# Pixie8888/R3DFSSeg

Hardware: AMD Instinct MI355X
Metric: episodes/sec S3DIS 2-way 5-shot 2048-pt (MPTI+attention, train step: forward+backward+grad all-reduce+Adam) (higher is better)
Workload: dtype f32 (index-free GEMMs -- self-attention, 1x1 convolutions, weight gradients, the EdgeConv backward's edge GEMMs -- as bf16x3 split products on the bf16 MFMA with fp32 accumulate; every index-deciding result: fp32)

## Files before the change

include/r3d.h:

```cpp
#ifndef R3D_H
#define R3D_H
#include <stdint.h>

#ifdef __cplusplus
extern "C" {
#endif

const char* r3d_last_error_string(void);
int r3d_abi_version(void);
int r3d_debug_poison_lds(unsigned pattern, unsigned* sink , void* stream);
int r3d_debug_set_cg_spmv_lds_min_blocks(int min_blocks);
int r3d_set_matrix_arith(int mode);
int r3d_get_matrix_arith(void);
int r3d_debug_set_gemm_bx3(int mask);

int r3d_cm_to_pm(const float* in , int B, int C, int N, float* out , long ld, void* stream);
int r3d_pm_to_cm(const float* in , long ld, int B, int C, int N, float* out , void* stream);
int r3d_pm_to_cm_pitched(const float* in, long ld, int B, int C, int N, float* out , long pitch, void* stream);
long r3d_cm_pitch(int N);
int r3d_copy_cols(const float* src, long ld_src, float* dst, long ld_dst, long M, int C, void* stream);

int r3d_sqnorm(const float* x, long ldx, long rows, int C, float* out, void* stream);
long r3d_knn_norm_ws_words(int B, int N);
int r3d_knn_topk(const float* x, long ldx, const float* x_cm, int B, int N, int C, int k, int mode,
// ... 38 lines not shown
                                int32_t* ws, long ws_words, long ws_stride, int flags, void* stream);

long r3d_lp_ws_words(int n_cap, int kp1);
int r3d_lp_ws_offsets(int n_cap, int kp1, long* out6);
int r3d_label_propagate(const float* nodes, long ldn, int D, const int32_t* nbr, int kp1, const float* Y,
                        const int32_t* n_dev, const int32_t* n_proto_dev, int n_cap, float sigma, float alpha,
                        int max_iter, float tol, float* Z, int32_t* ws, long ws_words, int32_t* stats_out, void* stream);

int r3d_label_propagate_batched(int n_ep, const float* nodes, long ldn, int D, const int32_t* nbr, int kp1, const float* Y,
                                const int32_t* n_dev, const int32_t* n_proto_dev, long desc_stride, int n_cap, float sigma,
                                float alpha, int max_iter, float tol, float* Z, int32_t* ws, long ws_words, long ws_stride,
                                int32_t* stats_out, long stats_stride, void* stream);
long r3d_graph_weights_verify_words(int n_cap, int kp1);
int r3d_graph_weights_verify(int n_ep, const float* nodes, long ldn, int D, const int32_t* n_dev, long desc_stride, int n_cap,
                             int kp1, float sigma, int32_t* ws, long ws_words, long ws_stride, float* scratch,
                             int32_t* mismatch_out, void* stream);

int r3d_label_propagate_solve_batched(int n_ep, const float* Y, const int32_t* n_dev, long desc_stride, int n_cap, int kp1,
                                      float alpha, int max_iter, float tol, float* Z, int32_t* ws, long ws_words,
                                      long ws_stride, int32_t* stats_out, long stats_stride, void* stream);

int r3d_graph_set_lp_budget(void* graph, void* graph_exec, int budget, int* n_cg);

int r3d_query_logits_ce(const float* Z, const int32_t* n_proto_dev, int n_q, int N, int n_classes,
                        const int64_t* labels , float* logits ,
                        float* loss_out , int32_t* pred_out , void* stream);

int r3d_query_logits_ce_batched(int n_ep, const float* Z, long z_ep_rows, const int32_t* n_proto_dev, long desc_stride, int n_q,
                                int N, int n_classes, const int64_t* labels, float* logits, float* loss_out, int32_t* pred_out,
                                void* stream);

int r3d_pointwise_conv_acc(const float* X, long ldx, const float* W, long M, int K, int Co, const float* scale,
                           const float* shift, int act, float* Out, long ldo, void* stream);
long r3d_pointwise_conv_stats_ws_words(long M, int Co);
int r3d_pointwise_conv_stats(const float* X, long ldx, const float* W, long M, int K, int Co, float* Out, long ldo,
                             float* sums_out , float* ws, void* stream);
int r3d_pointwise_conv_stats2(const float* X, long ldx, const float* W, long M, int K, int Co, float* Out, long ldo,
                              long M_first, float* sums_a , float* sums_b , float* ws, void* stream);
int r3d_pointwise_conv_stats_seg(const float* X, long ldx, const float* W, long M, int K, int Co, float* Out, long ldo,
                                 long rows_a, long rows_b, float* sums_out, float* ws, void* stream);
int r3d_colreduce(const float* part , int chunks, int C, float* sums_out , void* stream);
int r3d_colreduce_seg(const float* part, int count_a, int count_b, int n_seg, int C, float* sums_out , void* stream);
long r3d_colstats_ws_words(long M, int C);
int r3d_colstats(const float* X, long ldx, const float* DY, long lddy, long M, int C, int mode, const float* scale,
                 const float* shift, const float* mean, const float* invstd, int act, float* sums_out ,
                 float* ws, void* stream);
int r3d_bn_fold(const float* sums, double count, int C, const float* gamma, const float* beta, float eps,
                float momentum, float* running_mean , float* running_var , float* mean, float* invstd,
                float* scale, float* shift, float* rec , const int32_t* rec_index_dev , long rec_stride,
                void* stream);
long r3d_colstats_seg_ws_words(long M, int C, long rows_a, long rows_b);
int r3d_colstats_seg(const float* X, long ldx, const float* DY, long lddy, long M, int C, long rows_a, long rows_b, int mode,
                     const float* scale, const float* shift, const float* mean, const float* invstd, long bn_stride, int act,
                     float* sums_out , float* ws, void* stream);
int r3d_bn_fold_seg(const float* sums , int n_seg, double count_a, double count_b, int C, const float* gamma,
                    const float* beta, float eps, float momentum, float* running_mean , float* running_var ,
                    float* mean, float* invstd, float* scale, float* shift, long bn_stride, float* rec ,
                    const int32_t* rec_index_dev , long rec_stride, void* stream);
int r3d_affine_act_seg(const float* Z, long ldz, long M, int C, long rows_a, long rows_b, const float* scale, const float* shift,
                       long bn_stride, int act, float* Y, long ldy, void* stream);
int r3d_bn_bwd_apply_seg(const float* Z, long ldz, const float* DY, long lddy, long M, int C, long rows_a, long rows_b,
                         const float* scale, const float* shift, const float* mean, const float* invstd, long bn_stride, int act,
                         const float* sums , double count_a, double count_b, float* DZ, long lddz, void* stream);
int r3d_bn_running_update(const float* rec, int n_records, long rec_stride, int C, float momentum,
                          const float* bias , float* running_mean,
                          float* running_var, void* stream);
int r3d_affine_act(const float* Z, long ldz, long M, int C, const float* scale, const float* shift, int act, float* Y,
                   long ldy, void* stream);
int r3d_bn_bwd_apply(const float* Z, long ldz, const float* DY, long lddy, long M, int C, const float* scale,
                     const float* shift, const float* mean, const float* invstd, int act, const float* sums,
                     double count, float* DZ, long lddz, void* stream);
long r3d_gemm_tn_ws_words(long M, int Ca, int Cb);
int r3d_gemm_tn(const float* A, long lda, const float* B, long ldb, long M, int Ca, int Cb, float alpha, float* out,
                int accumulate, float* ws, void* stream);
int r3d_add_cols(const float* src, long ld_src, float* dst, long ld_dst, long M, int C, void* stream);

long r3d_edgeconv_train_ws_words(int B, int N);
int r3d_edge_stats1(const float* PQ, const int32_t* idx, int B, int N, int K, int clouds_a, int clouds_b,
                    float* sums_out , float* esum , float* ws,
                    void* stream);
int r3d_edgeconv_train_fwd_minmax(const float* PQ, const int32_t* idx, const float* s1, const float* t1, long bn_stride,
                                  const float* W2, int B, int N, int K, int clouds_a, int clouds_b, float* zmax, float* zmin,
                                  int32_t* argmax, int32_t* argmin, float* sums_out , float* ws, void* stream);
int r3d_edge_select(float* zmax , const float* zmin, int32_t* argmax ,
                    const int32_t* argmin, const float* s2, const float* t2, long bn_stride, long M, long rows_a, long rows_b,
                    float* out, long ldo, void* stream);
long r3d_edge_reverse_ws_words(int B, int N, int K);
int r3d_edge_reverse(const int32_t* idx, int B, int N, int K, int32_t* rev_ws, long ws_words, void* stream);
int r3d_edgeconv_bwd(const float* PQ, const int32_t* idx, const float* s1, const float* t1, const float* mean1,
                     const float* invstd1, const float* W2, const float* s2, const float* t2, const float* mean2,
                     const float* invstd2, long bn_stride, const float* bn2_sums, const float* dout, long lddo,
                     const int32_t* argmax, const float* zwin , const float* esum , int B, int N, int K,
                     int clouds_a, int clouds_b, float* DY1 , float* BE ,
                     const int32_t* rev_ws , float* dW2, float* bn1_sums, float* dPQ,
                     float* ws, void* stream);

int r3d_attention_fwd_train(const float* qkv, long ld, int B, int N, float* out, long ldo, float* lse_out, float p_drop,
                            unsigned seed, const unsigned* seed_dev, float* ws , void* stream);
int r3d_attention_bwd(const float* qkv, long ld, int B, int N, const float* O, long ldo, const float* dO, long lddo,
                      const float* lse, float p_drop, unsigned seed, const unsigned* seed_dev, float q_scale, float* dqkv,
                      long ldd, float* ws , void* stream);
int r3d_attention_bwd_ws(const float* qkv, long ld, int B, int N, const float* O, long ldo, const float* dO, long lddo,
                         const float* lse, float p_drop, unsigned seed, const unsigned* seed_dev, float q_scale,
                         float* dqkv, long ldd, float* ws, int ws_holds_packed_qkv, void* stream);

long r3d_attention_ws_words_ep(int B, int N, int seed_group);
int r3d_attention_fwd_train_ep(const float* qkv, long ld, int B, int N, float* out, long ldo, float* lse_out, float p_drop,
                               unsigned seed, const unsigned* seed_dev, int seed_group, float* ws, void* stream);
int r3d_attention_bwd_ep(const float* qkv, long ld, int B, int N, const float* O, long ldo, const float* dO, long lddo,
                         const float* lse, float p_drop, unsigned seed, const unsigned* seed_dev, int seed_group, float q_scale,
                         float* dqkv, long ldd, float* ws, int ws_holds_packed_qkv, void* stream);

long r3d_attention_ws_words_ep_d(int B, int N, int seed_group, int D);
int r3d_attention_fwd_train_ep_d(const float* qkv, long ld, int B, int N, float* out, long ldo, float* lse_out, float p_drop,
                                 unsigned seed, const unsigned* seed_dev, int seed_group, int D, float* ws, void* stream);
int r3d_attention_bwd_ep_d(const float* qkv, long ld, int B, int N, const float* O, long ldo, const float* dO, long lddo,
                           const float* lse, float p_drop, unsigned seed, const unsigned* seed_dev, int seed_group, int D,
                           float q_scale, float* dqkv, long ldd, float* ws, int ws_holds_packed_qkv, void* stream);

int r3d_ce_grad(const float* Z, const int32_t* n_proto_dev, int n_cap, int n_query_pts, int n_classes,
                const int64_t* labels, const float* gscale_dev, float* G, void* stream);
int r3d_label_propagate_bwd(const float* nodes, long ldn, int D, int kp1, const float* Z, const float* G,
                            const int32_t* n_dev, int n_cap, float sigma, float alpha, int max_iter, float tol, float* lam,
                            float* dnodes, long ldd, int32_t* ws, long ws_words, int32_t* stats_out, void* stream);
int r3d_head_prototypes_bwd(const float* dnodes, long ldd, int n_way, int k_shot, int N, int D, int n_query_pts,
                            const int32_t* desc, const int32_t* assign, const int32_t* cluster_count, const int32_t* ws,
                            float* dsfeat, long lds_, float* dqfeat, long ldq, void* stream);

int r3d_ce_grad_batched(int n_ep, const float* Z, const int32_t* n_proto_dev, long desc_stride, int n_cap, int n_query_pts,
                        int n_classes, const int64_t* labels, const float* gscale_dev, float* G, void* stream);
int r3d_label_propagate_bwd_batched(int n_ep, const float* nodes, long ldn, int D, int kp1, const float* Z, const float* G,
                                    const int32_t* n_dev, long desc_stride, int n_cap, float sigma, float alpha, int max_iter,
                                    float tol, float* lam, float* dnodes, long ldd, int32_t* ws, long ws_words, long ws_stride,
                                    int32_t* stats_out, long stats_stride, void* stream);
int r3d_head_prototypes_bwd_batched(int n_ep, const float* dnodes, long ldd, long nodes_ep_rows, int n_way, int k_shot, int N,
                                    int D, int n_query_pts, const int32_t* desc, long desc_stride, const int32_t* assign,
                                    long assign_stride, const int32_t* cluster_count, long ccount_stride, const int32_t* ws,
                                    long ws_stride, float* dsfeat, long lds_, long dsfeat_ep_rows, float* dqfeat, long ldq,
                                    long dqfeat_ep_rows, void* stream);

long r3d_contrast_ws_words(int n_way, int k_shot, int N);
int r3d_contrast_fwd(const float* feat, long ldf, int D, const int32_t* support_y, const int32_t* support_flag, int n_way,
                     int k_shot, int N, const float* W, const float* bias, float temp, float* loss_out, float* ws,
                     long ws_words, void* stream);
int r3d_contrast_bwd(int D, int n_way, int k_shot, int N, const float* gscale_dev, float* dfeat, long ldd, float* dW,
                     float* db, float* ws, void* stream);
int r3d_contrast_fwd_batched(int n_ep, const float* feat, long ldf, long feat_ep_rows, int D, const int32_t* support_y,
                             const int32_t* support_flag, int n_way, int k_shot, int N, const float* W, const float* bias,
                             float temp, float* loss_out, float* ws, long ws_words, long ws_stride, void* stream);
int r3d_contrast_bwd_batched(int n_ep, int D, int n_way, int k_shot, int N, const float* gscale_dev, float* dfeat, long ldd,
                             long dfeat_ep_rows, float* dW, float* db, float* ws, long ws_stride, void* stream);
int r3d_train_metrics_batched(int n_ep, const int32_t* pred, const int64_t* query_y, const int64_t* gt_query_y, int n_query_pts,
                              const float* Z, long z_ep_rows, const int32_t* desc, long desc_stride, const int32_t* proto_ws,
                              long pws_stride, const int32_t* assign, long assign_stride, const int32_t* gt_support_y, int n_way,
                              int k_shot, int N, float* out4 , void* stream);
int r3d_train_metrics(const int32_t* pred, const int64_t* query_y, const int64_t* gt_query_y, int n_query_pts, const float* Z,
                      const int32_t* desc, const int32_t* proto_ws, const int32_t* assign, const int32_t* gt_support_y,
                      int n_way, int k_shot, int N, float* out4, void* stream);

long r3d_clean_ws_words(int n_way, int k_shot);
int r3d_clean_shot_detect(const float* feat , long ldf, int D, const float* support_x ,
                          int Cin, const int32_t* support_y, int n_way, int k_shot, int N, int32_t* shot_keep,
                          float* dbg_cos_sum , int32_t* ws, void* stream);

int r3d_clean_shot_detect_batched(int n_ep, const float* feat, long ldf, long feat_ep_rows, int D, const float* support_x,
                                  int Cin, const int32_t* support_y, int n_way, int k_shot, int N, int32_t* shot_keep,
// ... 14 lines not shown
```

r3dfsseg_amd/_lib.py:

```python
import ctypes
import os
import re

_HERE = os.path.dirname(os.path.abspath(__file__))
LIB_PATH = os.environ.get("R3D_LIB") or os.path.join(_HERE, "libr3d_hip.so")
HEADER_PATH = os.path.join(os.path.dirname(_HERE), "include", "r3d.h")

c_f = ctypes.c_void_p
c_i = ctypes.c_int
c_l = ctypes.c_long
c_fl = ctypes.c_float
c_d = ctypes.c_double
c_u = ctypes.c_uint

_SIGS = {
    "r3d_last_error_string": (ctypes.c_char_p, []),
    "r3d_abi_version": (c_i, []),
    "r3d_cm_to_pm": (c_i, [c_f, c_i, c_i, c_i, c_f, c_l, c_f]),
    "r3d_pm_to_cm": (c_i, [c_f, c_l, c_i, c_i, c_i, c_f, c_f]),
    "r3d_pm_to_cm_pitched": (c_i, [c_f, c_l, c_i, c_i, c_i, c_f, c_l, c_f]),
    "r3d_cm_pitch": (c_l, [c_i]),
    "r3d_copy_cols": (c_i, [c_f, c_l, c_f, c_l, c_l, c_i, c_f]),
    "r3d_sqnorm": (c_i, [c_f, c_l, c_l, c_i, c_f, c_f]),
    "r3d_knn_topk": (c_i, [c_f, c_l, c_f, c_i, c_i, c_i, c_i, c_i, c_f, c_f, c_f, c_f, c_f, c_f, c_f]),
    "r3d_pointwise_conv": (c_i, [c_f, c_l, c_f, c_l, c_i, c_i, c_f, c_f, c_i, c_f, c_l, c_f]),
    "r3d_edgeconv_fwd": (c_i, [c_f, c_f, c_f, c_f, c_f, c_f, c_l, c_i, c_i, c_i, c_f, c_f]),
    "r3d_attention_ws_words": (c_l, [c_i, c_i]),
    "r3d_knn_norm_ws_words": (c_l, [c_i, c_i]),
    "r3d_attention_fwd": (c_i, [c_f, c_l, c_i, c_i, c_f, c_l, c_f, c_f, c_f]),
    "r3d_head_desc_words": (c_i, []),
    "r3d_debug_poison_lds": (c_i, [c_u, c_f, c_f]),
    "r3d_debug_set_cg_spmv_lds_min_blocks": (c_i, [c_i]),
    "r3d_debug_set_gemm_bx3": (c_i, [c_i]),
    "r3d_set_matrix_arith": (c_i, [c_i]),
    "r3d_get_matrix_arith": (c_i, []),
    "r3d_head_max_k": (c_i, []),
    "r3d_fps_sample_count_table": (c_i, [c_i, c_i, c_f, c_f]),
    "r3d_head_proto_ws_words": (c_l, [c_i, c_i, c_i]),
    "r3d_head_proto_ws_offsets": (c_i, [c_i, c_i, c_i, ctypes.POINTER(c_l)]),
    "r3d_head_prototypes": (c_i, [c_f, c_f, c_f, c_l, c_f, c_f, c_l, c_i, c_i, c_i, c_i, c_i, c_i, c_f, c_l,
                                  c_f, c_f, c_f, c_f, c_f, c_l, c_i, c_f]),
    "r3d_lp_ws_words": (c_l, [c_i, c_i]),
    "r3d_lp_ws_offsets": (c_i, [c_i, c_i, ctypes.POINTER(c_l)]),
    "r3d_label_propagate": (c_i, [c_f, c_l, c_i, c_f, c_i, c_f, c_f, c_f, c_i, c_fl, c_fl, c_i, c_fl, c_f, c_f,
                                  c_l, c_f, c_f]),
    "r3d_graph_set_lp_budget": (c_i, [c_f, c_f, c_i, ctypes.POINTER(c_i)]),
    "r3d_pointwise_conv_acc": (c_i, [c_f, c_l, c_f, c_l, c_i, c_i, c_f, c_f, c_i, c_f, c_l, c_f]),
    "r3d_edgeconv_train_fwd_minmax": (c_i, [c_f, c_f, c_f, c_f, c_l, c_f, c_i, c_i, c_i, c_i, c_i, c_f, c_f, c_f, c_f, c_f, c_f, c_f]),
    "r3d_edge_select": (c_i, [c_f, c_f, c_f, c_f, c_f, c_f, c_l, c_l, c_l, c_l, c_f, c_l, c_f]),
    "r3d_pointwise_conv_stats_ws_words": (c_l, [c_l, c_i]),
    "r3d_pointwise_conv_stats": (c_i, [c_f, c_l, c_f, c_l, c_i, c_i, c_f, c_l, c_f, c_f, c_f]),
    "r3d_pointwise_conv_stats2": (c_i, [c_f, c_l, c_f, c_l, c_i, c_i, c_f, c_l, c_l, c_f, c_f, c_f, c_f]),
    "r3d_colreduce": (c_i, [c_f, c_i, c_i, c_f, c_f]),
    "r3d_colstats_ws_words": (c_l, [c_l, c_i]),
    "r3d_colstats": (c_i, [c_f, c_l, c_f, c_l, c_l, c_i, c_i, c_f, c_f, c_f, c_f, c_i, c_f, c_f, c_f]),
    "r3d_bn_fold": (c_i, [c_f, c_d, c_i, c_f, c_f, c_fl, c_fl, c_f, c_f, c_f, c_f, c_f, c_f, c_f, c_f, c_l, c_f]),
    "r3d_bn_running_update": (c_i, [c_f, c_i, c_l, c_i, c_fl, c_f, c_f, c_f, c_f]),
    "r3d_affine_act": (c_i, [c_f, c_l, c_l, c_i, c_f, c_f, c_i, c_f, c_l, c_f]),
    "r3d_bn_bwd_apply": (c_i, [c_f, c_l, c_f, c_l, c_l, c_i, c_f, c_f, c_f, c_f, c_i, c_f, c_d, c_f, c_l, c_f]),
    "r3d_gemm_tn_ws_words": (c_l, [c_l, c_i, c_i]),
    "r3d_gemm_tn": (c_i, [c_f, c_l, c_f, c_l, c_l, c_i, c_i, c_fl, c_f, c_i, c_f, c_f]),
    "r3d_add_cols": (c_i, [c_f, c_l, c_f, c_l, c_l, c_i, c_f]),
    "r3d_edgeconv_train_ws_words": (c_l, [c_i, c_i]),
    "r3d_edge_stats1": (c_i, [c_f, c_f, c_i, c_i, c_i, c_i, c_i, c_f, c_f, c_f, c_f]),
    "r3d_edge_reverse_ws_words": (c_l, [c_i, c_i, c_i]),
    "r3d_edge_reverse": (c_i, [c_f, c_i, c_i, c_i, c_f, c_l, c_f]),
    "r3d_edgeconv_bwd": (c_i, [c_f] * 11 + [c_l, c_f, c_f, c_l, c_f, c_f, c_f, c_i, c_i, c_i, c_i, c_i, c_f, c_f, c_f, c_f, c_f, c_f, c_f, c_f]),
    "r3d_attention_fwd_train": (c_i, [c_f, c_l, c_i, c_i, c_f, c_l, c_f, c_fl, c_u, c_f, c_f, c_f]),
    "r3d_attention_bwd": (c_i, [c_f, c_l, c_i, c_i, c_f, c_l, c_f, c_l, c_f, c_fl, c_u, c_f, c_fl, c_f, c_l, c_f, c_f]),
    "r3d_attention_bwd_ws": (c_i, [c_f, c_l, c_i, c_i, c_f, c_l, c_f, c_l, c_f, c_fl, c_u, c_f, c_fl, c_f, c_l, c_f, c_i, c_f]),
    "r3d_ce_grad": (c_i, [c_f, c_f, c_i, c_i, c_i, c_f, c_f, c_f, c_f]),
    "r3d_label_propagate_bwd": (c_i, [c_f, c_l, c_i, c_i, c_f, c_f, c_f, c_i, c_fl, c_fl, c_i, c_fl, c_f, c_f, c_l, c_f, c_l, c_f, c_f]),
    "r3d_head_prototypes_bwd": (c_i, [c_f, c_l, c_i, c_i, c_i, c_i, c_i, c_f, c_f, c_f, c_f, c_f, c_l, c_f, c_l, c_f]),
    "r3d_contrast_ws_words": (c_l, [c_i, c_i, c_i]),
    "r3d_contrast_fwd": (c_i, [c_f, c_l, c_i, c_f, c_f, c_i, c_i, c_i, c_f, c_f, c_fl, c_f, c_f, c_l, c_f]),
    "r3d_contrast_bwd": (c_i, [c_i, c_i, c_i, c_i, c_f, c_f, c_l, c_f, c_f, c_f, c_f]),
    "r3d_train_metrics": (c_i, [c_f, c_f, c_f, c_i, c_f, c_f, c_f, c_f, c_f, c_i, c_i, c_i, c_f, c_f]),
    "r3d_clean_ws_words": (c_l, [c_i, c_i]),
    "r3d_clean_shot_detect": (c_i, [c_f, c_l, c_i, c_f, c_i, c_f, c_i, c_i, c_i, c_f, c_f, c_f, c_f]),
    "r3d_protonet_head": (c_i, [c_f, c_l, c_f, c_l, c_i, c_f, c_i, c_i, c_i, c_i, c_i, c_fl, c_f, c_f, c_f]),
    "r3d_miou_accumulate": (c_i, [c_f, c_f, c_l, c_f, c_i, c_i, c_f, c_f]),
    "r3d_query_logits_ce": (c_i, [c_f, c_f, c_i, c_i, c_i, c_f, c_f, c_f, c_f, c_f]),
    "r3d_knn_topk_batched": (c_i, [c_f, c_l, c_f, c_i, c_i, c_i, c_i, c_i, c_f, c_i, c_f, c_l, c_f, c_f, c_f, c_f]),
    "r3d_knn_ws_words": (c_l, [c_i, c_i, c_i, c_i, c_i]),
    "r3d_debug_set_knn_bf16_threshold": (c_i, [c_i]),
    "r3d_debug_set_knn_bf16_filter": (c_i, [c_i]),
    "r3d_set_wpack_in_capture": (c_i, [c_i]),
    "r3d_pointwise_conv_stats_seg": (c_i, [c_f, c_l, c_f, c_l, c_i, c_i, c_f, c_l, c_l, c_l, c_f, c_f, c_f]),
    "r3d_colreduce_seg": (c_i, [c_f, c_i, c_i, c_i, c_i, c_f, c_f]),
    "r3d_colstats_seg_ws_words": (c_l, [c_l, c_i, c_l, c_l]),
    "r3d_colstats_seg": (c_i, [c_f, c_l, c_f, c_l, c_l, c_i, c_l, c_l, c_i, c_f, c_f, c_f, c_f, c_l, c_i, c_f, c_f, c_f]),
    "r3d_bn_fold_seg": (c_i, [c_f, c_i, c_d, c_d, c_i, c_f, c_f, c_fl, c_fl, c_f, c_f, c_f, c_f, c_f, c_f, c_l, c_f, c_f, c_l, c_f]),
    "r3d_affine_act_seg": (c_i, [c_f, c_l, c_l, c_i, c_l, c_l, c_f, c_f, c_l, c_i, c_f, c_l, c_f]),
    "r3d_bn_bwd_apply_seg": (c_i, [c_f, c_l, c_f, c_l, c_l, c_i, c_l, c_l, c_f, c_f, c_f, c_f, c_l, c_i, c_f, c_d, c_d, c_f, c_l, c_f]),
    "r3d_attention_ws_words_ep": (c_l, [c_i, c_i, c_i]),
    "r3d_attention_fwd_train_ep": (c_i, [c_f, c_l, c_i, c_i, c_f, c_l, c_f, c_fl, c_u, c_f, c_i, c_f, c_f]),
    "r3d_attention_bwd_ep": (c_i, [c_f, c_l, c_i, c_i, c_f, c_l, c_f, c_l, c_f, c_fl, c_u, c_f, c_i, c_fl, c_f, c_l, c_f, c_i, c_f]),
    "r3d_attention_ws_words_ep_d": (c_l, [c_i, c_i, c_i, c_i]),
    "r3d_attention_fwd_train_ep_d": (c_i, [c_f, c_l, c_i, c_i, c_f, c_l, c_f, c_fl, c_u, c_f, c_i, c_i, c_f, c_f]),
    "r3d_attention_bwd_ep_d": (c_i, [c_f, c_l, c_i, c_i, c_f, c_l, c_f, c_l, c_f, c_fl, c_u, c_f, c_i, c_i, c_fl, c_f, c_l, c_f, c_i,
                                     c_f]),
    "r3d_head_prototypes_batched": (c_i, [c_i, c_i, c_f, c_l, c_f, c_l, c_f, c_l, c_l, c_f, c_l, c_l, c_i, c_i, c_i, c_i, c_i, c_i,
                                          c_f, c_l, c_l, c_f, c_f, c_l, c_f, c_l, c_f, c_l, c_f, c_l, c_l, c_i, c_f]),
    "r3d_head_prototypes_bwd_batched": (c_i, [c_i, c_f, c_l, c_l, c_i, c_i, c_i, c_i, c_i, c_f, c_l, c_f, c_l, c_f, c_l, c_f, c_l,
                                              c_f, c_l, c_l, c_f, c_l, c_l, c_f]),
    "r3d_graph_weights_verify_words": (c_l, [c_i, c_i]),
    "r3d_graph_weights_verify": (c_i, [c_i, c_f, c_l, c_i, c_f, c_l, c_i, c_i, c_fl, c_f, c_l, c_l, c_f, c_f, c_f]),
    "r3d_label_propagate_solve_batched": (c_i, [c_i, c_f, c_f, c_l, c_i, c_i, c_fl, c_i, c_fl, c_f, c_f, c_l, c_l, c_f, c_l, c_f]),
    "r3d_label_propagate_batched": (c_i, [c_i, c_f, c_l, c_i, c_f, c_i, c_f, c_f, c_f, c_l, c_i, c_fl, c_fl, c_i, c_fl, c_f, c_f,
                                          c_l, c_l, c_f, c_l, c_f]),
    "r3d_label_propagate_bwd_batched": (c_i, [c_i, c_f, c_l, c_i, c_i, c_f, c_f, c_f, c_l, c_i, c_fl, c_fl, c_i, c_fl, c_f, c_f,
                                              c_l, c_f, c_l, c_l, c_f, c_l, c_f]),
    "r3d_ce_grad_batched": (c_i, [c_i, c_f, c_f, c_l, c_i, c_i, c_i, c_f, c_f, c_f, c_f]),
    "r3d_query_logits_ce_batched": (c_i, [c_i, c_f, c_l, c_f, c_l, c_i, c_i, c_i, c_f, c_f, c_f, c_f, c_f]),
    "r3d_contrast_fwd_batched": (c_i, [c_i, c_f, c_l, c_l, c_i, c_f, c_f, c_i, c_i, c_i, c_f, c_f, c_fl, c_f, c_f, c_l, c_l, c_f]),
    "r3d_contrast_bwd_batched": (c_i, [c_i, c_i, c_i, c_i, c_i, c_f, c_f, c_l, c_l, c_f, c_f, c_f, c_l, c_f]),
    "r3d_train_metrics_batched": (c_i, [c_i, c_f, c_f, c_f, c_i, c_f, c_l, c_f, c_l, c_f, c_l, c_f, c_l, c_f, c_i, c_i, c_i, c_f, c_f]),
    "r3d_clean_shot_detect_batched": (c_i, [c_i, c_f, c_l, c_l, c_i, c_f, c_i, c_f, c_i, c_i, c_i, c_f, c_f, c_f, c_l, c_f]),
}

_lib = None


def header_symbols():
    txt = open(HEADER_PATH).read()
    txt = re.sub(r"/\*.*?\*/", "", txt, flags=re.S)
    return sorted(set(re.findall(r"\b(r3d_[a-z0-9_]+)\s*\(", txt)))


ABI_VERSION = 5

# ... 63 lines not shown
```

r3dfsseg_amd/csrc/edgeconv_train.hip:

```cpp
#include <stdlib.h>
#include "edge_tile.h"

#define ET_LD 65
#define ET_MAXBLK 1024
#define EC_CHUNK 32

static __device__ __forceinline__ float lrelu(float v) { return v > 0.f ? v : 0.2f * v; }

struct EcGeom {
  int N, cpc;
  __host__ __device__ static EcGeom make(int N) { return EcGeom{N, (N + EC_CHUNK - 1) / EC_CHUNK}; }
  __device__ void range(int chunk, int& cloud, int& p0, int& p1) const {
    cloud = __builtin_amdgcn_readfirstlane(chunk / cpc);
    p0 = __builtin_amdgcn_readfirstlane(cloud * N + (chunk - cloud * cpc) * EC_CHUNK);
    p1 = __builtin_amdgcn_readfirstlane(min(p0 + EC_CHUNK, (cloud + 1) * N));
  }
};
static __device__ __forceinline__ int ec_seg(const r3d_segmap& cs, int cloud) {
  return __builtin_amdgcn_readfirstlane(cs.seg_of_row32(cloud));
}

template <int RT>
__global__ __launch_bounds__(256) void r3d_edge_stats1_kernel(const float* __restrict__ PQ, const int* __restrict__ idx,
                                                              EcGeom gm, int n_chunks, float* __restrict__ part,
// ... 224 lines not shown
  int tid2 = threadIdx.x;
  asm volatile("" : "+v"(tid2));
  const int w2 = tid2 >> 6, n2 = tid2 & 15, g2 = (tid2 >> 4) & 3;
  float* mypart = part_dw + (long)blockIdx.x * 4096;
#pragma unroll
  for (int i = 0; i < 4; ++i)
    *(float4*)(mypart + (16 * w2 + 4 * g2 + i) * 64 + 4 * n2) = float4{dw[0][i], dw[1][i], dw[2][i], dw[3][i]};
}

template <int RT>
__global__ __launch_bounds__(256) void r3d_edgeconv_train_fwd2_kernel(
    const float* __restrict__ PQ, const int* __restrict__ idx, const float* __restrict__ s1, const float* __restrict__ t1,
    long bn_stride, const float* __restrict__ W2, EcGeom gm, r3d_segmap cs , int n_chunks,
    int* __restrict__ argmax_out, float* __restrict__ zmax_out, float* __restrict__ zmin_out, int* __restrict__ argmin_out,
    float* __restrict__ part ) {
  constexpr int K = 4 * RT, R = 16 * RT;
  extern __shared__ __attribute__((aligned(16))) float smem[];
  float* H = smem;
  float* Z = smem + R * E2_LD;
  const int tid = threadIdx.x, lane = tid & 63, w = tid >> 6;
  const int n = lane & 15, g = lane >> 4;
  const int c = 16 * w + n;
  const int N = gm.N;
  float Bz[16];
#pragma unroll
  for (int s = 0; s < 16; ++s) Bz[s] = W2[c * 64 + 16 * g + s];
  for (int item = blockIdx.x; item < n_chunks; item += gridDim.x) {
    const int chunk = r3d_xcd_swizzle(item, n_chunks);
    int cloud, p0, p1;
    gm.range(chunk, cloud, p0, p1);
    const long cloud0 = (long)cloud * N;
    const long bo = (long)ec_seg(cs, cloud) * bn_stride;
    const float sc1 = s1[bo + lane], sh1 = t1[bo + lane];
    float za = 0.f, zb = 0.f;
    for (int pt0_ = p0; pt0_ < p1; pt0_ += E2_PTS) {
      const long pt0 = pt0_;
      {
        const int my_idx = min(max(idx[(pt0 + w) * K + min(lane, K - 1)], 0), N - 1);
        const float q = PQ[(pt0 + w) * 128 + 64 + lane];
        float pv[K];
#pragma unroll
        for (int t = 0; t < K; ++t) pv[t] = PQ[(cloud0 + __builtin_amdgcn_readlane(my_idx, t)) * 128 + lane];
        float* hrow = H + (K * w) * E2_LD + lane;
#pragma unroll
        for (int t = 0; t < K; ++t) hrow[t * E2_LD] = lrelu(sc1 * (pv[t] + q) + sh1);
      }
      __syncthreads();
      f32x4 acc[RT];
      e2_rowgemm<RT>(H, Bz, n, g, acc);
#pragma unroll
      for (int t = 0; t < RT; ++t) {
#pragma unroll
        for (int i = 0; i < 4; ++i) {
          const float z = acc[t][i];
          za += z;
          zb += z * z;
          Z[(16 * t + 4 * g + i) * E2_LD + c] = z;
        }
      }
      __syncthreads();
      {
        const float* zp = Z + (K * w) * E2_LD + lane;
        float zx = zp[0], zn = zx;
        int ax = 0, an = 0;
#pragma unroll
        for (int t = 1; t < K; ++t) {
          const float z = zp[t * E2_LD];
          if (z > zx) { zx = z; ax = t; }
          if (z < zn) { zn = z; an = t; }
        }
        const long o = (pt0 + w) * 64 + lane;
        zmax_out[o] = zx;
        zmin_out[o] = zn;
        argmax_out[o] = ax;
        argmin_out[o] = an;
      }
    }
    za += __shfl_xor(za, 16); zb += __shfl_xor(zb, 16);
    za += __shfl_xor(za, 32); zb += __shfl_xor(zb, 32);
    if (g == 0) {
      part[((long)chunk * 2 + 0) * 64 + c] = za;
      part[((long)chunk * 2 + 1) * 64 + c] = zb;
    }
  }
}

#define RV_RANGE 256
#define RV_CAP 12288
__global__ __launch_bounds__(1024) void r3d_edge_reverse_kernel(const int* __restrict__ idx, int N, int K, int n_clouds,
                                                                int* __restrict__ rev_ptr, int* __restrict__ rev) {
  __shared__ int cnt[RV_RANGE];
  __shared__ int off[RV_RANGE + 1];
  __shared__ int cur[RV_RANGE];
  __shared__ int buf[RV_CAP];
  __shared__ int wsum[16];
  __shared__ int below_s, b_s;
  const int tid = threadIdx.x, lane = tid & 63, w = tid >> 6;
  const int cloud = blockIdx.y;
  const int r0 = blockIdx.x * RV_RANGE, nr = min(RV_RANGE, N - r0);
  const long E = (long)N * K, gbase = (long)cloud * E;
  const int* lst = idx + gbase;
  if (tid < RV_RANGE) cnt[tid] = 0;
  if (tid == 0) below_s = 0;
  __syncthreads();
  int my_below = 0;
  for (long e0 = tid; e0 < E; e0 += 8 * 1024) {
    int jv[8];
#pragma unroll
    for (int u = 0; u < 8; ++u) jv[u] = lst[min(e0 + 1024 * u, E - 1)];
#pragma unroll
    for (int u = 0; u < 8; ++u) {
      const int j = min(max(jv[u], 0), N - 1) - r0;
      if (e0 + 1024 * u < E) {
        if (j < 0) ++my_below;
        else if (j < nr) atomicAdd(&cnt[j], 1);
      }
    }
  }
#pragma unroll
  for (int o = 32; o > 0; o >>= 1) my_below += __shfl_xor(my_below, o);
  if (lane == 0) atomicAdd(&below_s, my_below);
  __syncthreads();
  if (tid < RV_RANGE) {
    const int v = tid < nr ? cnt[tid] : 0;
    int x = v;
#pragma unroll
    for (int o = 1; o < 64; o <<= 1) {
      const int y = __shfl_up(x, o);
      if (lane >= o) x += y;
    }
    if (lane == 63) wsum[w] = x;
    cur[tid] = x - v;
  }
  __syncthreads();
  if (tid < RV_RANGE) {
    int wb = 0;
    for (int q = 0; q < w; ++q) wb += wsum[q];
    off[tid] = cur[tid] + wb;
  }
  if (tid == 0) {
    int t = 0;
    for (int q = 0; q < RV_RANGE / 64; ++q) t += wsum[q];
    off[RV_RANGE] = t;
  }
  __syncthreads();
  const long seg0 = gbase + below_s;
  if (tid < nr) rev_ptr[(long)cloud * N + r0 + tid] = (int)(seg0 + off[tid]);
  if (cloud == n_clouds - 1 && r0 + nr == N && tid == 0) rev_ptr[(long)n_clouds * N] = (int)((long)n_clouds * E);
  int a = 0;
  while (a < nr) {
    if (tid == 0) {
      int b = nr;
      if (off[nr] - off[a] > RV_CAP) {
        int lo = a, hi = nr;
        while (lo < hi) {
          const int mid = (lo + hi + 1) >> 1;
          if (off[mid] - off[a] <= RV_CAP) lo = mid; else hi = mid - 1;
        }
        b = lo;
      }
      b_s = b;
    }
    __syncthreads();
    const int b = b_s;
    if (b == a) {
      long outp = seg0 + off[a];
// ... 108 lines not shown
    const int src1 = __builtin_amdgcn_readfirstlane(min(e0 + 63, e_end - 1) / K);
    int pos = 0;
    for (int g = src0; g <= src1; ++g)
      if (ok && src == g) pos = atomicAdd(&mine[j], 1);
    if (ok) rev[gbase + pos] = (int)(gbase + e);
  }
}

template <int RT>
__global__ __launch_bounds__(256) void r3d_edgeconv_bwd2_kernel(
    const float* __restrict__ PQ, const float* __restrict__ s1, const float* __restrict__ mean1,
    const float* __restrict__ invstd1, long bn_stride, const float* __restrict__ bn1_sums ,
    const float* __restrict__ DY1, const float* __restrict__ BE, const float* __restrict__ esum ,
    const int* __restrict__ rev_ptr, const int* __restrict__ rev,
    int e_off, EcGeom gm, r3d_segmap cs , int n_chunks, float* __restrict__ dPQ ) {
  constexpr int K = 4 * RT;
  const int lane = threadIdx.x & 63, w = threadIdx.x >> 6;
  for (int item = blockIdx.x; item < n_chunks; item += gridDim.x) {
    const int chunk = r3d_xcd_swizzle(item, n_chunks);
    int cloud, p0, p1;
    gm.range(chunk, cloud, p0, p1);
    const int seg = ec_seg(cs, cloud);
    const long bo = (long)seg * bn_stride;
    const double E = (double)cs.seg_rows(seg) * gm.N * K;
    const float sc1 = s1[bo + lane], mu1 = mean1[bo + lane], is1 = invstd1[bo + lane];
    const float n1 = (float)((double)bn1_sums[(long)seg * 128 + lane] / E), n2 = (float)((double)bn1_sums[(long)seg * 128 + 64 + lane] / E);
    for (int pt_ = p0 + w; pt_ < p1; pt_ += 4) {
      const long pt = pt_;
      const int rb = rev_ptr[pt], re = rev_ptr[pt + 1];
      const float pj = PQ[pt * 128 + lane];
      const float bs = BE[pt * 128 + lane];
      const float es = esum ? (esum[pt * 64 + lane] - (float)K * mu1) * is1 : BE[pt * 128 + 64 + lane];
      float asum = 0.f, gsum = 0.f;
      for (int e0 = rb; e0 < re; e0 += 16) {
        const int my_e = rev[min(e0 + min(lane, 15), re - 1)];
        float dv[16], qv[16];
#pragma unroll
        for (int t = 0; t < 16; ++t) {
          const int e = __builtin_amdgcn_readlane(my_e, t) - e_off;
          dv[t] = DY1[(long)e * 64 + lane];
          qv[t] = PQ[(long)(e / K) * 128 + 64 + lane];
        }
#pragma unroll
        for (int t = 0; t < 16; ++t) {
          const bool ok = e0 + t < re;
          asum += r3d_keep(dv[t], ok);
          gsum += r3d_keep(qv[t], ok);
        }
      }
      const float cj = (float)(re - rb);
      dPQ[pt * 128 + lane] = sc1 * (asum - cj * n1 - n2 * (is1 * (cj * (pj - mu1) + gsum)));
      dPQ[pt * 128 + 64 + lane] = sc1 * (bs - (float)K * n1 - n2 * es);
    }
  }
}

static int et_check(const char* fn, int B, int N, int K, int clouds_a, int clouds_b) {
  if (B <= 0 || N <= 0 || N % E2_PTS != 0 || K < 4 || K > 32 || K % 4 != 0) {
    r3d_set_error("%s: unsupported shape B=%d N=%d K=%d (N %% 4 == 0, K %% 4 == 0, 4..32)", fn, B, N, K);
    return R3D_ERR_ARG;
  }
  const r3d_segmap cs{clouds_a, clouds_b};
  if (!cs.covers(B)) {
    r3d_set_error("%s: %d clouds are not whole segments of %d + %d clouds", fn, B, clouds_a, clouds_b);
    return R3D_ERR_ARG;
  }
  if ((long)B * N * K >= 0x7fffffffL) {
    r3d_set_error("%s: B*N*K = %ld edges exceed the 31-bit edge ids", fn, (long)B * N * K);
    return R3D_ERR_ARG;
  }
  return 0;
}
static int et_chunks(int B, int N) { return B * EcGeom::make(N).cpc; }
static int et_grid8(int n_chunks, int cap) { return n_chunks <= cap ? n_chunks : (cap >= 8 ? cap & ~7 : cap); }

extern "C" long r3d_edgeconv_train_ws_words(int B, int N) { return (long)ET_MAXBLK * 4096 + (long)et_chunks(B, N) * 128 + 64; }

static void et_reduce_chunks(const float* part, int N, int clouds_a, int clouds_b, int n_seg, float* out, hipStream_t st) {
  const int cpc = EcGeom::make(N).cpc;
  hipLaunchKernelGGL(r3d_part_reduce_kernel, dim3(128 / 64, n_seg), dim3(1024), 0, st, part, clouds_a * cpc, clouds_b * cpc, 128,
                     out, 128L, 128, (float*)nullptr, 0L);
}

extern "C" int r3d_edge_stats1(const float* PQ, const int32_t* idx, int B, int N, int K, int clouds_a, int clouds_b,
                               float* sums_out, float* esum, float* ws, void* stream) {
  R3D_REQUIRE(PQ && idx && sums_out && ws, "r3d_edge_stats1: null pointer");
  int rc = et_check("r3d_edge_stats1", B, N, K, clouds_a, clouds_b);
  if (rc) return rc;
  hipStream_t st = (hipStream_t)stream;
  const EcGeom gm = EcGeom::make(N);
  const int n_chunks = et_chunks(B, N);
  const int grid = et_grid8(n_chunks, 2048);
#define E2_CASE(RT) \
  case RT: hipLaunchKernelGGL(r3d_edge_stats1_kernel<RT>, dim3(grid), dim3(256), 0, st, PQ, idx, gm, n_chunks, ws, esum); break
  switch (K / 4) {
    E2_CASE(1); E2_CASE(2); E2_CASE(3); E2_CASE(4); E2_CASE(5); E2_CASE(6); E2_CASE(7); E2_CASE(8);
  }
#undef E2_CASE
  et_reduce_chunks(ws, N, clouds_a, clouds_b, r3d_segmap{clouds_a, clouds_b}.n_seg(B), sums_out, st);
  R3D_LAUNCH_CHECK("r3d_edge_stats1");
  return R3D_OK;
}

template <int RT>
static int fwd2_launch_rt(int n_chunks, hipStream_t st, const float* PQ, const int32_t* idx, const float* s1, const float* t1,
                          long bn_stride, const float* W2, EcGeom gm, r3d_segmap cs, int32_t* argmax, float* zmax, float* zmin,
                          int32_t* argmin, float* ws) {
  const size_t lds = sizeof(float) * ((size_t)2 * 16 * RT * E2_LD);
  static int resident = 0;
  if (!resident) {
    resident = e2_resident_blocks(r3d_edgeconv_train_fwd2_kernel<RT>, lds, ET_MAXBLK);
    R3D_REQUIRE(resident > 0, "r3d_edgeconv_train_fwd_minmax: cannot reserve %zu B of LDS", lds);
  }
  const int grid = et_grid8(n_chunks, resident);
  hipLaunchKernelGGL(r3d_edgeconv_train_fwd2_kernel<RT>, dim3(grid), dim3(256), lds, st, PQ, idx, s1, t1, bn_stride, W2, gm, cs,
                     n_chunks, argmax, zmax, zmin, argmin, ws);
  return R3D_OK;
}

extern "C" int r3d_edgeconv_train_fwd_minmax(const float* PQ, const int32_t* idx, const float* s1, const float* t1,
                                             long bn_stride, const float* W2, int B, int N, int K, int clouds_a, int clouds_b,
                                             float* zmax, float* zmin, int32_t* argmax, int32_t* argmin, float* sums_out,
                                             float* ws, void* stream) {
  R3D_REQUIRE(PQ && idx && s1 && t1 && W2 && zmax && zmin && argmax && argmin && sums_out && ws,
              "r3d_edgeconv_train_fwd_minmax: null pointer");
  int rc = et_check("r3d_edgeconv_train_fwd_minmax", B, N, K, clouds_a, clouds_b);
  if (rc) return rc;
  hipStream_t st = (hipStream_t)stream;
  const EcGeom gm = EcGeom::make(N);
  const r3d_segmap cs{clouds_a, clouds_b};
  const int n_chunks = et_chunks(B, N);
#define E2_CASE(RT)                                                                                                    \
  case RT:                                                                                                             \
    rc = fwd2_launch_rt<RT>(n_chunks, st, PQ, idx, s1, t1, bn_stride, W2, gm, cs, argmax, zmax, zmin, argmin, ws);      \
    break
  switch (K / 4) {
    E2_CASE(1); E2_CASE(2); E2_CASE(3); E2_CASE(4); E2_CASE(5); E2_CASE(6); E2_CASE(7); E2_CASE(8);
  }
#undef E2_CASE
  if (rc) return rc;
  et_reduce_chunks(ws, N, clouds_a, clouds_b, cs.n_seg(B), sums_out, st);
  R3D_LAUNCH_CHECK("r3d_edgeconv_train_fwd_minmax");
  return R3D_OK;
}

__global__ void r3d_edge_select_kernel(float* __restrict__ zmax, const float* __restrict__ zmin, int* __restrict__ argmax,
                                       const int* __restrict__ argmin, const float* __restrict__ s2,
                                       const float* __restrict__ t2, long bn_stride, r3d_segmap sm , long M,
                                       float* __restrict__ out, long ldo) {
  const long i = (long)blockIdx.x * blockDim.x + threadIdx.x;
  if (i >= M * 64) return;
  const int c = (int)(i & 63);
  const long m = (long)__builtin_amdgcn_readfirstlane((int)(i >> 6));
  const long bo = (long)__builtin_amdgcn_readfirstlane(sm.seg_of_row32((int)m)) * bn_stride + c;
  const float sc = s2[bo];
  const bool up = sc >= 0.f;
  const float z = up ? zmax[i] : zmin[i];
  if (!up) { zmax[i] = z; argmax[i] = argmin[i]; }
  out[m * ldo + c] = lrelu(sc * z + t2[bo]);
}
extern "C" int r3d_edge_select(float* zmax, const float* zmin, int32_t* argmax, const int32_t* argmin, const float* s2,
                               const float* t2, long bn_stride, long M, long rows_a, long rows_b, float* out, long ldo,
                               void* stream) {
  R3D_REQUIRE(zmax && zmin && argmax && argmin && s2 && t2 && out && M > 0 && ldo >= 64, "r3d_edge_select: bad arguments");
  const r3d_segmap sm{rows_a, rows_b};
  R3D_REQUIRE(sm.covers(M), "r3d_edge_select: %ld rows are not whole segments of %ld + %ld rows", M, rows_a, rows_b);
  hipLaunchKernelGGL(r3d_edge_select_kernel, dim3(r3d_cdiv(M * 64, 256)), dim3(256), 0, (hipStream_t)stream, zmax, zmin,
                     argmax, argmin, s2, t2, bn_stride, sm, M, out, ldo);
  R3D_LAUNCH_CHECK("r3d_edge_select");
  return R3D_OK;
}

template <int RT>
static int bwd1_launch_rt(int n_chunks, hipStream_t st, const float* PQ, const int32_t* idx, EcBn bn, const float* W2,
                          const float* bn2_sums, const float* dout, long lddo, const int32_t* argmax, EcGeom gm, r3d_segmap cs,
                          float* DY1, float* BE, float* part_dw, float* part_bn, int* grid_out) {
  const size_t lds = sizeof(float) * ((size_t)2 * 16 * RT * E2_LD + 2 * E2_PTS * 64 + 6 * 64);
  static int resident = 0;
  if (!resident) {
    resident = e2_resident_blocks(r3d_edgeconv_bwd1_kernel<RT>, lds, ET_MAXBLK);
    R3D_REQUIRE(resident > 0, "r3d_edgeconv_bwd: cannot reserve %zu B of LDS", lds);
  }
  const int grid = et_grid8(n_chunks, resident);
  hipLaunchKernelGGL(r3d_edgeconv_bwd1_kernel<RT>, dim3(grid), dim3(256), lds, st, PQ, idx, bn, W2, bn2_sums, dout, lddo, argmax,
                     gm, cs, n_chunks, DY1, BE, part_dw, part_bn);
  *grid_out = grid;
  return R3D_OK;
}

template <int RT>
static int bwd1_bx3_launch_rt(int n_chunks, hipStream_t st, const float* PQ, const int32_t* idx, EcBn bn, const float* W2,
                              const float* bn2_sums, const float* dout, long lddo, const int32_t* argmax, const float* zwin,
                              EcGeom gm, r3d_segmap cs, float* DY1, float* BE, float* part_dw, float* part_bn, int* grid_out) {
  static int resident = 0;
  if (!resident) {
    resident = e2_resident_blocks(r3d_edgeconv_bwd1_bx3_kernel<RT>, EB_LDS_BYTES, ET_MAXBLK / 2);
    R3D_REQUIRE(resident > 0, "r3d_edgeconv_bwd: cannot reserve %d B of LDS", (int)EB_LDS_BYTES);
  }
  const int grid = et_grid8(n_chunks, resident);
  hipLaunchKernelGGL(r3d_edgeconv_bwd1_bx3_kernel<RT>, dim3(grid), dim3(256), EB_LDS_BYTES, st, PQ, idx, bn, W2, bn2_sums, dout,
                     lddo, argmax, zwin, gm, cs, n_chunks, DY1, BE, part_dw, part_bn);
  *grid_out = grid;
  return R3D_OK;
}

extern "C" long r3d_edge_reverse_ws_words(int B, int N, int K) { return (long)B * N + 1 + (long)B * N * K + 16; }
extern "C" int r3d_edge_reverse(const int32_t* idx, int B, int N, int K, int32_t* rev_ws, long ws_words, void* stream) {
  R3D_REQUIRE(idx && rev_ws, "r3d_edge_reverse: null pointer");
  R3D_REQUIRE(B > 0 && B <= 65535 && N > 0 && K > 0 && (long)B * N * K < 0x7fffffffL, "r3d_edge_reverse: bad shape B=%d N=%d K=%d",
              B, N, K);
  R3D_REQUIRE(ws_words >= r3d_edge_reverse_ws_words(B, N, K), "r3d_edge_reverse: workspace of %ld words is shorter than "
              "r3d_edge_reverse_ws_words(%d, %d, %d)", ws_words, B, N, K);
  const size_t ro_lds = sizeof(int) * (size_t)RO_WAVES * N;
  static const bool ro_off = getenv("R3D_EDGE_REVERSE_SORT") != nullptr;
  if (!ro_off && ro_lds <= 144 * 1024 && (long)N * K >= 64 * RO_WAVES) {
    static size_t attr = 0;
    if (ro_lds > attr) {
// ... 66 lines not shown
```

Measured before the change: 389.0.

## Add software-pipelined EdgeConv forward kernel with buffer-load gathers and single LDS tile

Adds a new EdgeConv training forward kernel that walks point tiles with a three-stage cursor. It prefetches the next tile's neighbor indices, gathered rows and BN scale/shift while the current tile's MFMA row-GEMM and min/max selection run. Neighbor rows are gathered with raw buffer loads relative to a per-cloud resource descriptor. The Z tile is kept in a per-wave LDS region so the argmax/argmin step needs only wave-level barriers, and the H buffer is single-buffered to reduce LDS use. A debug switch and a size guard fall back to the legacy kernel.

```diff
diff --git a/include/r3d.h b/include/r3d.h
--- a/include/r3d.h
+++ b/include/r3d.h
@@ -144,6 +144,7 @@
 int r3d_edgeconv_train_fwd_minmax(const float* PQ, const int32_t* idx, const float* s1, const float* t1, long bn_stride,
                                   const float* W2, int B, int N, int K, int clouds_a, int clouds_b, float* zmax, float* zmin,
                                   int32_t* argmax, int32_t* argmin, float* sums_out , float* ws, void* stream);
+int r3d_debug_set_edgeconv_fwd_legacy(int on);
 int r3d_edge_select(float* zmax , const float* zmin, int32_t* argmax ,
                     const int32_t* argmin, const float* s2, const float* t2, long bn_stride, long M, long rows_a, long rows_b,
                     float* out, long ldo, void* stream);
diff --git a/r3dfsseg_amd/_lib.py b/r3dfsseg_amd/_lib.py
--- a/r3dfsseg_amd/_lib.py
+++ b/r3dfsseg_amd/_lib.py
@@ -47,6 +47,7 @@
     "r3d_graph_set_lp_budget": (c_i, [c_f, c_f, c_i, ctypes.POINTER(c_i)]),
     "r3d_pointwise_conv_acc": (c_i, [c_f, c_l, c_f, c_l, c_i, c_i, c_f, c_f, c_i, c_f, c_l, c_f]),
     "r3d_edgeconv_train_fwd_minmax": (c_i, [c_f, c_f, c_f, c_f, c_l, c_f, c_i, c_i, c_i, c_i, c_i, c_f, c_f, c_f, c_f, c_f, c_f, c_f]),
+    "r3d_debug_set_edgeconv_fwd_legacy": (c_i, [c_i]),
     "r3d_edge_select": (c_i, [c_f, c_f, c_f, c_f, c_f, c_f, c_l, c_l, c_l, c_l, c_f, c_l, c_f]),
     "r3d_pointwise_conv_stats_ws_words": (c_l, [c_l, c_i]),
     "r3d_pointwise_conv_stats": (c_i, [c_f, c_l, c_f, c_l, c_i, c_i, c_f, c_l, c_f, c_f, c_f]),
diff --git a/r3dfsseg_amd/csrc/edgeconv_train.hip b/r3dfsseg_amd/csrc/edgeconv_train.hip
--- a/r3dfsseg_amd/csrc/edgeconv_train.hip
+++ b/r3dfsseg_amd/csrc/edgeconv_train.hip
@@ -330,6 +330,147 @@
       part[((long)chunk * 2 + 0) * 64 + c] = za;
       part[((long)chunk * 2 + 1) * 64 + c] = zb;
     }
+  }
+}
+
+struct EcCursor {
+  int item, chunk, cloud, p0, p1, pt;
+  __device__ void first(const EcGeom& gm, int n_chunks, int it) {
+    item = it;
+    if (item < n_chunks) {
+      chunk = r3d_xcd_swizzle(item, n_chunks);
+      gm.range(chunk, cloud, p0, p1);
+      pt = p0;
+    }
+  }
+  __device__ bool valid(int n_chunks) const { return item < n_chunks; }
+  __device__ void next(const EcGeom& gm, int n_chunks) {
+    if (item >= n_chunks) return;
+    pt += E2_PTS;
+    if (pt >= p1) first(gm, n_chunks, item + (int)gridDim.x);
+  }
+};
+
+static __device__ __forceinline__ __amdgpu_buffer_rsrc_t ec_cloud_rows(const float* PQ, int cloud, int N) {
+  return __builtin_amdgcn_make_buffer_rsrc((void*)(PQ + (long)cloud * N * 128), 0, N * 512, 0x00020000);
+}
+static __device__ __forceinline__ float ec_row_load(__amdgpu_buffer_rsrc_t rs, int row, int lane_bytes) {
+  return __builtin_bit_cast(float, __builtin_amdgcn_raw_buffer_load_b32(rs, lane_bytes, row * 512, 0));
+}
+
+template <int RT>
+__global__ __launch_bounds__(256) __attribute__((amdgpu_waves_per_eu(3))) void r3d_edgeconv_train_fwd3_kernel(
+    const float* __restrict__ PQ, const int* __restrict__ idx, const float* __restrict__ s1, const float* __restrict__ t1,
+    long bn_stride, const float* __restrict__ W2, EcGeom gm, r3d_segmap cs , int n_chunks,
+    int* __restrict__ argmax_out, float* __restrict__ zmax_out, float* __restrict__ zmin_out, int* __restrict__ argmin_out,
+    float* __restrict__ part ) {
+  constexpr int K = 4 * RT, R = 16 * RT, ZLD = R + 4;
+  extern __shared__ __attribute__((aligned(16))) float smem[];
+  const int tid = threadIdx.x, lane = tid & 63;
+  const int w = __builtin_amdgcn_readfirstlane(tid >> 6);
+  const int n = lane & 15, g = lane >> 4;
+  const int c = 16 * w + n;
+  const int N = gm.N;
+  float* H = smem;
+  float* Zt = smem + R * E2_LD + w * 16 * ZLD + n * ZLD;
+  float Bz[16];
+#pragma unroll
+  for (int s = 0; s < 16; ++s) Bz[s] = W2[c * 64 + 16 * g + s];
+  EcCursor cur, nxt, nx2;
+  cur.first(gm, n_chunks, blockIdx.x);
+  if (!cur.valid(n_chunks)) return;
+  nxt = cur;
+  nxt.next(gm, n_chunks);
+  nx2 = nxt;
+  nx2.next(gm, n_chunks);
+  auto list = [&](int pt) { return idx[((long)pt + w) * K + min(lane, K - 1)]; };
+  float pv[K], q;
+  auto rows = [&](const EcCursor& u, int my_idx) {
+    my_idx = min(max(my_idx, 0), N - 1);
+    const __amdgpu_buffer_rsrc_t rs = ec_cloud_rows(PQ, u.cloud, N);
+    q = PQ[((long)u.pt + w) * 128 + 64 + lane];
+#pragma unroll
+    for (int t = 0; t < K; ++t) pv[t] = ec_row_load(rs, __builtin_amdgcn_readlane(my_idx, t), 4 * lane);
+  };
+  rows(cur, list(cur.pt));
+  int idx1 = list(nxt.valid(n_chunks) ? nxt.pt : cur.pt);
+  float sc1, sh1;
+  {
+    const long bo = (long)ec_seg(cs, cur.cloud) * bn_stride;
+    sc1 = s1[bo + lane];
+    sh1 = t1[bo + lane];
+  }
+  float za = 0.f, zb = 0.f;
+  for (;;) {
+    {
+      float* hrow = H + (K * w) * E2_LD + lane;
+#pragma unroll
+      for (int t = 0; t < K; ++t) hrow[t * E2_LD] = lrelu(sc1 * (pv[t] + q) + sh1);
+    }
+    __syncthreads();
+    const bool has1 = nxt.valid(n_chunks), has2 = nx2.valid(n_chunks);
+    const int idx2 = list(has2 ? nx2.pt : cur.pt);
+    const EcCursor& un = has1 ? nxt : cur;
+    rows(un, idx1);
+    const long bo = (long)ec_seg(cs, un.cloud) * bn_stride;
+    const float sc1n = s1[bo + lane], sh1n = t1[bo + lane];
+    __builtin_amdgcn_sched_barrier(0);
+    f32x4 acc[RT];
+    e2_rowgemm<RT>(H, Bz, n, g, acc);
+#pragma unroll
+    for (int t = 0; t < RT; ++t) {
+#pragma unroll
+      for (int i = 0; i < 4; ++i) {
+        const float z = acc[t][i];
+        za += z;
+        zb += z * z;
+      }
+      *(f32x4*)(Zt + 16 * t + 4 * g) = acc[t];
+    }
+    __builtin_amdgcn_fence(__ATOMIC_RELEASE, "wavefront");
+    __builtin_amdgcn_wave_barrier();
+    {
+      const float* zp = Zt + K * g;
+      float zv[K];
+#pragma unroll
+      for (int s = 0; s < RT; ++s) {
+        const f32x4 v = *(const f32x4*)(zp + 4 * s);
+        zv[4 * s] = v[0]; zv[4 * s + 1] = v[1]; zv[4 * s + 2] = v[2]; zv[4 * s + 3] = v[3];
+      }
+      float zx = zv[0], zn = zx;
+      int ax = 0, an = 0;
+#pragma unroll
+      for (int t = 1; t < K; ++t) {
+        const float z = zv[t];
+        if (z > zx) { zx = z; ax = t; }
+        if (z < zn) { zn = z; an = t; }
+      }
+      const long o = ((long)cur.pt + g) * 64 + c;
+      zmax_out[o] = zx;
+      zmin_out[o] = zn;
+      argmax_out[o] = ax;
+      argmin_out[o] = an;
+    }
+    __builtin_amdgcn_fence(__ATOMIC_RELEASE, "wavefront");
+    __builtin_amdgcn_wave_barrier();
+    if (!has1 || nxt.item != cur.item) {
+      za += __shfl_xor(za, 16); zb += __shfl_xor(zb, 16);
+      za += __shfl_xor(za, 32); zb += __shfl_xor(zb, 32);
+      if (g == 0) {
+        part[((long)cur.chunk * 2 + 0) * 64 + c] = za;
+        part[((long)cur.chunk * 2 + 1) * 64 + c] = zb;
+      }
+      za = 0.f;
+      zb = 0.f;
+    }
+    if (!has1) break;
+    __syncthreads();
+    cur = nxt;
+    nxt = nx2;
+    nx2.next(gm, n_chunks);
+    idx1 = idx2;
+    sc1 = sc1n;
+    sh1 = sh1n;
   }
 }
 
@@ -604,6 +745,14 @@
                      out, 128L, 128, (float*)nullptr, 0L);
 }
 
+static int g_ec_fwd_legacy = 0;
+extern "C" int r3d_debug_set_edgeconv_fwd_legacy(int on) {
+  const int old = g_ec_fwd_legacy;
+  g_ec_fwd_legacy = on ? 1 : 0;
+  return old;
+}
+static bool ec_fwd_legacy(int N) { return g_ec_fwd_legacy || (long)N * 512 > 0x7fffffffL; }
+
 extern "C" int r3d_edge_stats1(const float* PQ, const int32_t* idx, int B, int N, int K, int clouds_a, int clouds_b,
                                float* sums_out, float* esum, float* ws, void* stream) {
   R3D_REQUIRE(PQ && idx && sums_out && ws, "r3d_edge_stats1: null pointer");
@@ -640,6 +789,22 @@
   return R3D_OK;
 }
 
+template <int RT>
+static int fwd3_launch_rt(int n_chunks, hipStream_t st, const float* PQ, const int32_t* idx, const float* s1, const float* t1,
+                          long bn_stride, const float* W2, EcGeom gm, r3d_segmap cs, int32_t* argmax, float* zmax, float* zmin,
+                          int32_t* argmin, float* ws) {
+  const size_t lds = sizeof(float) * ((size_t)16 * RT * E2_LD + (size_t)4 * 16 * (16 * RT + 4));
+  static int resident = 0;
+  if (!resident) {
+    resident = e2_resident_blocks(r3d_edgeconv_train_fwd3_kernel<RT>, lds, ET_MAXBLK);
+    R3D_REQUIRE(resident > 0, "r3d_edgeconv_train_fwd_minmax: cannot reserve %zu B of LDS", lds);
+  }
+  const int grid = et_grid8(n_chunks, resident);
+  hipLaunchKernelGGL(r3d_edgeconv_train_fwd3_kernel<RT>, dim3(grid), dim3(256), lds, st, PQ, idx, s1, t1, bn_stride, W2, gm,
+                     cs, n_chunks, argmax, zmax, zmin, argmin, ws);
+  return R3D_OK;
+}
+
 extern "C" int r3d_edgeconv_train_fwd_minmax(const float* PQ, const int32_t* idx, const float* s1, const float* t1,
                                              long bn_stride, const float* W2, int B, int N, int K, int clouds_a, int clouds_b,
                                              float* zmax, float* zmin, int32_t* argmax, int32_t* argmin, float* sums_out,
@@ -652,9 +817,11 @@
   const EcGeom gm = EcGeom::make(N);
   const r3d_segmap cs{clouds_a, clouds_b};
   const int n_chunks = et_chunks(B, N);
+  const bool legacy = ec_fwd_legacy(N);
 #define E2_CASE(RT)                                                                                                    \
   case RT:                                                                                                             \
-    rc = fwd2_launch_rt<RT>(n_chunks, st, PQ, idx, s1, t1, bn_stride, W2, gm, cs, argmax, zmax, zmin, argmin, ws);      \
+    rc = legacy ? fwd2_launch_rt<RT>(n_chunks, st, PQ, idx, s1, t1, bn_stride, W2, gm, cs, argmax, zmax, zmin, argmin, ws) \
+       : fwd3_launch_rt<RT>(n_chunks, st, PQ, idx, s1, t1, bn_stride, W2, gm, cs, argmax, zmax, zmin, argmin, ws);        \
     break
   switch (K / 4) {
     E2_CASE(1); E2_CASE(2); E2_CASE(3); E2_CASE(4); E2_CASE(5); E2_CASE(6); E2_CASE(7); E2_CASE(8);
```

After: 389.5 (median of 6 runs). Within noise of the previous version (+0.1%).
